# FeatureBaseDB/featurebase

Measured on NVIDIA B200. Metric: set_ops_per_sec, higher is better.
Workload: dtype u64/u16 integer

## Files before the change

### featurebase_b200/csrc/fbgpu.cu

```cuda
#include <cuda_runtime.h>
#include <dlfcn.h>
#include <fcntl.h>
#include <sys/mman.h>
#include <sys/stat.h>
#include <unistd.h>
#include <stdarg.h>
#include <stdio.h>
#include <string.h>

#include <algorithm>
#include <condition_variable>
#include <map>
#include <memory>
#include <mutex>
#include <shared_mutex>
#include <atomic>
#include <deque>
#include <functional>
#include <string>
#include <thread>
#include <unordered_map>
#include <vector>

#include "../../include/fbgpu.h"
// ... 109 lines not shown
    cudaEvent_t ev0 = nullptr, ev1 = nullptr;
    DevBuf d_in, d_counts, d_bitmaps, d_info, d_emit_units, d_emit, d_rows, d_aux;
    PinBuf h_in, h_out;
    bool busy = false;
};

struct fbgpu_ctx {
    int device = 0;
    int sm_count = 148;
    std::shared_mutex store_mu;
    std::map<ViewKey, uint32_t> view_ids;
    std::vector<std::vector<int32_t>> shardmaps;
    std::vector<uint64_t> view_arr, view_other;
    std::vector<uint64_t> view_striped;
    std::vector<HostFrag> frags;
    std::vector<FragHdr> h_frags;
    std::vector<RowEnt> h_rows;
    std::vector<ContDesc> h_descs;
    RawBuf staging;
    uint64_t uploaded = 0;
    uint64_t dead_arena = 0;
    bool meta_dirty = false;
    bool tables_valid = false;
    bool dev_tables_valid = false;
    std::vector<std::pair<uint32_t, uint64_t>> dirty_shards;
    size_t dev_rows = 0, dev_descs = 0, dev_frags = 0;
    bool inspect_only = false;
    std::vector<ViewTab> t_views; std::vector<int32_t> t_flat; std::vector<RowTabEnt> t_rowtab;
    bool stripe_arrays = getenv("FBGPU_ARRAY_SORTED") == nullptr;
    long long unit_batch = [] { const char* e = getenv("FBGPU_UNIT_BATCH"); const long long n = e ? atoll(e) : 0; return n >= 16 ? (n / 16) * 16 : 16384ll; }();
    int gd_ctas_per_sm = 3;
    int pair_ctas_per_sm = 2;
    std::atomic<uint64_t> counters_pair_launches{0};
    DevBuf d_payload, d_views, d_shardmap, d_frags, d_rows, d_descs, d_rowtab;
    PinBuf bounce[2];
    uint32_t n_views_dev = 0;
    fbgpu_stats stats{};
    std::mutex ws_mu; std::condition_variable ws_cv;
    std::vector<std::unique_ptr<Workspace>> wss;
    std::mutex cnt_mu; fbgpu_counters counters{};
    void* comm = nullptr; int n_ranks = 1, rank = 0;
    Mailbox* mbox = nullptr; Mailbox* peers[kMaxRanks] = {}; DevBuf d_peers; bool p2p = false; bool peers_local = false; unsigned long long epoch = 0; std::mutex coll_mu;
    long long p2p_timeout_cycles = [] { const char* e = getenv("FBGPU_P2P_TIMEOUT_MS"); const long long ms = e ? atoll(e) : 2000; return (ms > 0 ? ms : 2000) * 2000000ll; }();
};

static StoreRef store_ref(fbgpu_ctx* c) {
    StoreRef s;
    s.views = (const ViewTab*)c->d_views.p; s.shardmap = (const int32_t*)c->d_shardmap.p; s.frags = (const FragHdr*)c->d_frags.p;
    s.rows = (const RowEnt*)c->d_rows.p; s.descs = (const ContDesc*)c->d_descs.p; s.payload = (const uint8_t*)c->d_payload.p; s.rowtab = (const RowTabEnt*)c->d_rowtab.p; s.n_views = c->n_views_dev;
    return s;
}

extern "C" int fbgpu_init(int32_t device_ordinal, fbgpu_ctx** out) try {
    if (!out) return fail(FBGPU_E_INVALID, "out is null");
    if (device_ordinal == FBGPU_DEVICE_NONE) {
        auto c = new fbgpu_ctx(); c->inspect_only = true; c->device = -1;
        *out = c;
        return FBGPU_OK;
    }
    int n = 0;
    CUDA_TRY(cudaGetDeviceCount(&n));
    if (device_ordinal < 0 || device_ordinal >= n) return fail(FBGPU_E_INVALID, "device ordinal %d out of range (%d devices)", device_ordinal, n);
    CUDA_TRY(cudaSetDevice(device_ordinal));
    auto c = new fbgpu_ctx();
    struct Guard { fbgpu_ctx* c; ~Guard() { if (c) fbgpu_shutdown(c); } } guard{ c };
    c->device = device_ordinal;
// ... 645 lines not shown
    if (!c || !out) return fail(FBGPU_E_INVALID, "null argument");
    std::shared_lock<std::shared_mutex> lk(c->store_mu);
    *out = c->stats;
    return 0;
} FBGPU_CATCH

static int compile_program(fbgpu_ctx* c, uint32_t index, const fbgpu_op* ops, int32_t n_ops, std::vector<DevOp>& out, int& depth) {
    Error err;
    ViewLookup lookup = [c, index](uint32_t field, uint32_t view) { return view_id_locked(c, ViewKey{ index, field, view }, false); };
    int rc = compile(ops, n_ops, lookup, out, depth, err);
    if (rc) return fail(rc, "%s", err.msg);
#ifndef FBGPU_WP_LEGACY_LOOP
    expand_push_row(out);
#endif
    return 0;
}

static void bump(fbgpu_ctx* c, uint64_t launches, float ms) {
    std::lock_guard<std::mutex> lk(c->cnt_mu);
    c->counters.kernel_launches += launches; c->counters.queries++; c->counters.last_query_gpu_ms = ms;
}

static int allreduce_u64(fbgpu_ctx* c, Workspace* w, void* dptr, size_t n) {
    if (!c->comm) return 0;
    std::lock_guard<std::mutex> lk(c->coll_mu);
    int r = g_nccl.AllReduce(dptr, dptr, n, kNcclUint64, kNcclSum, c->comm, w->stream);
    if (r != 0) return fail(FBGPU_E_COMM, "ncclAllReduce failed: %s", g_nccl.GetErrorString ? g_nccl.GetErrorString(r) : "?");
    return 0;
}

static std::vector<int2> find_batches(const std::vector<DevOp>& prog);
static int upload_inputs(Workspace* w, const std::vector<DevOp>& prog, const uint64_t* shards, int64_t n_shards, const DevOp** d_prog, const uint64_t** d_shards) {
    std::vector<int2> batches = find_batches(prog);
    size_t pb = prog.size() * sizeof(DevOp), sb = (size_t)n_shards * 8, bb = batches.size() * sizeof(int2), tot = pb + sb + bb;
    if (w->h_in.ensure(tot + 16)) return FBGPU_E_NOMEM;
    if (w->d_in.ensure(pb + sb + 16)) return FBGPU_E_NOMEM;
    if (w->d_aux.ensure(bb + 16)) return FBGPU_E_NOMEM;
    if (pb) memcpy(w->h_in.p, prog.data(), pb);
    if (sb) memcpy((uint8_t*)w->h_in.p + pb, shards, sb);
    if (bb) memcpy((uint8_t*)w->h_in.p + pb + sb, batches.data(), bb);
    if (pb + sb) CUDA_TRY(cudaMemcpyAsync(w->d_in.p, w->h_in.p, pb + sb, cudaMemcpyHostToDevice, w->stream));
    if (bb) CUDA_TRY(cudaMemcpyAsync(w->d_aux.p, (uint8_t*)w->h_in.p + pb + sb, bb, cudaMemcpyHostToDevice, w->stream));
    *d_prog = (const DevOp*)w->d_in.p; *d_shards = (const uint64_t*)((uint8_t*)w->d_in.p + pb);
    return 0;
}

static std::vector<int2> find_batches(const std::vector<DevOp>& prog) {
    std::vector<int2> b;
    for (size_t k = 0; k < prog.size();) {
        uint8_t o = prog[k].op;
        if (o == D_OR_ROW || o == D_ANDNOT_ROW || o == D_XOR_ROW) { size_t e = k + 1; while (e < prog.size() && prog[e].op == o) e++; b.push_back(make_int2((int)k, (int)e)); k = e; }
        else k++;
    }
    return b;
}

static int launch_eval(fbgpu_ctx* c, Workspace* w, const std::vector<DevOp>& prog, const DevOp* d_prog, int depth, const uint64_t* d_shards, long long n_units, EvalOut out) {
    if (n_units <= 0) return 0;
    const int n_ops = (int)prog.size();
    std::vector<int2> batches = find_batches(prog);
    size_t staged_rows = 0; for (auto& b : batches) staged_rows += (size_t)(b.y - b.x);
    if (!out.info && n_ops <= kWpMaxOps && depth <= kWpMaxDepth && !getenv("FBGPU_NO_WORDPAR")) {
        uint64_t arr = 0, other = 0, striped = 0;
        for (const DevOp& o : prog) if (o.op >= D_PUSH_ROW && o.op <= D_ORANDNOT_ROW && o.op != D_PUSH_EMPTY && o.fv < c->view_arr.size()) { arr += c->view_arr[o.fv]; other += c->view_other[o.fv]; striped += c->view_striped[o.fv]; }
        if (striped == 0 && ((other > 0 && arr * 8 <= other) || getenv("FBGPU_FORCE_WORDPAR") != nullptr)) {
            long long blocks = n_units * kWpBlocksPerUnit;
            long long grid = std::min<long long>(blocks, (long long)c->sm_count * std::max(FBGPU_WP_MIN_BLOCKS, 8) * 2);
            eval_wordpar_kernel<<<(unsigned)grid, kWpThreads, 0, w->stream>>>(store_ref(c), d_prog, n_ops, d_shards, n_units, out);
            CUDA_TRY(cudaGetLastError());
            return 0;
        }
    }
    const bool staged = getenv("FBGPU_STAGED") && n_ops <= kStagedMaxOps && staged_rows >= 4;
    const int2* d_batches = reinterpret_cast<const int2*>(w->d_aux.p);
    if (staged) {
        int ctas = 2;
        if (const char* e = getenv("FBGPU_STAGE_CTAS")) ctas = std::max(1, std::min(4, atoi(e)));
        const size_t per_cta = 233472 / ctas - 1024 - 5888;
        size_t stack = (size_t)(depth + 1) * 8192;
        if (stack + 2 * 8192 <= per_cta) {
            uint32_t stg = (uint32_t)(((per_cta - stack) / 2) & ~size_t(127));
            long long grid = std::min<long long>(n_units, (long long)c->sm_count * ctas);
            size_t smem = stack + 2 * (size_t)stg;
            eval_staged_kernel<<<(unsigned)grid, kEvalThreads, smem, w->stream>>>(store_ref(c), d_prog, n_ops, depth, d_batches, (int)batches.size(), stg, d_shards, n_units, out);
            CUDA_TRY(cudaGetLastError());
            return 0;
        }
    }
    size_t smem = (size_t)(depth + 1) * 8192;
    int per_sm = std::max(1, (int)std::min<size_t>(std::min(FBGPU_EVAL_MIN_BLOCKS, 2048 / kEvalThreads), (227 * 1024) / (smem + 3 * 1024 + 512)));
    long long grid = std::min<long long>(n_units, (long long)c->sm_count * per_sm);
    eval_kernel<<<(unsigned)grid, kEvalThreads, smem, w->stream>>>(store_ref(c), d_prog, n_ops, depth, d_batches, (int)batches.size(), d_shards, n_units, out);
    CUDA_TRY(cudaGetLastError());
    return 0;
}

static bool contiguous_shards(const uint64_t* shards, int64_t n) {
    for (int64_t i = 1; i < n; i++) if (shards[i] != shards[0] + (uint64_t)i) return false;
    return n > 0;
}

static int count_impl(fbgpu_ctx* c, uint32_t index, const fbgpu_op* ops, int32_t n_ops, const uint64_t* shards, int64_t n_shards,
                      uint64_t* out_total, uint64_t* out_per_shard, bool collective) {
    if (!c || !out_total || n_shards < 0 || (n_shards && !shards)) return fail(FBGPU_E_INVALID, "null argument");
    USE_DEVICE(c);
    std::shared_lock<std::shared_mutex> lk;
    int rc = lock_committed(c, lk); if (rc) return rc;
    std::vector<DevOp> prog; int depth = 1;
    rc = compile_program(c, index, ops, n_ops, prog, depth); if (rc) return rc;
    WsLease lease(c); Workspace* w = lease.w;
    const DevOp* d_prog; const uint64_t* d_shards;
    rc = upload_inputs(w, prog, shards, n_shards, &d_prog, &d_shards); if (rc) return rc;
    const size_t nper = out_per_shard ? (size_t)n_shards : 0, nc = 1 + nper + 3;
    if (w->d_counts.ensure(nc * 8)) return FBGPU_E_NOMEM;
    if (w->h_out.ensure(nc * 8)) return FBGPU_E_NOMEM;
    CUDA_TRY(cudaMemsetAsync(w->d_counts.p, 0, nc * 8, w->stream));
    unsigned long long* d_total = (unsigned long long*)w->d_counts.p;
    unsigned long long* d_per = out_per_shard ? d_total + 1 : nullptr;
    long long n_units = (long long)n_shards * kSlotsPerRow;
    std::unique_lock<std::mutex> coll_lk(c->coll_mu, std::defer_lock);
    FuseReduce fr{};
    coll_lk.lock();
    const bool p2p = c->p2p && collective;
    if (!p2p) coll_lk.unlock();
    if (p2p) {
// ... 742 lines not shown
    StoreRef st{};
    st.views = c->t_views.data(); st.shardmap = c->t_flat.data(); st.frags = c->h_frags.data(); st.rows = c->h_rows.data(); st.descs = c->h_descs.data();
    st.payload = c->staging.p; st.rowtab = c->t_rowtab.data(); st.n_views = (uint32_t)c->t_views.size();
    uint32_t fv = index == 0xffffffffu ? field : view_id_locked(c, ViewKey{ index, field, view }, false);
    Resolved r = resolve(st, fv, shard, row, slot);
    *out_type = 0; *out_card = 0; *out_runs = 0; *out_len = 0;
    if (r.ptr == nullptr) return FBGPU_OK;
    *out_type = r.typ; *out_card = r.card; *out_runs = r.cnt;
    const uint64_t bytes = r.typ == kArray ? (((uint64_t)r.card * 2 + 15) & ~15ull) : r.typ == kBitmap ? 8192 : (((uint64_t)r.cnt * 4 + 15) & ~15ull);
    *out_len = bytes;
    if (bytes > cap || !out_payload) return fail(FBGPU_E_NOSPACE, "payload needs %llu bytes", (unsigned long long)bytes);
    if ((const uint8_t*)r.ptr + bytes > c->staging.p + c->staging.len) return fail(FBGPU_E_INVALID, "descriptor points outside the payload arena");
    memcpy(out_payload, r.ptr, bytes);
    return FBGPU_OK;
} FBGPU_CATCH

extern "C" int fbgpu_debug_compile(fbgpu_ctx* c, uint32_t index, const fbgpu_op* ops, int32_t n_ops, uint8_t* out, int32_t cap_ops, int32_t* out_n, int32_t* out_depth) try {
    if (!c || !out_n || !out_depth) return fail(FBGPU_E_INVALID, "null argument");
    std::shared_lock<std::shared_mutex> lk(c->store_mu);
    std::vector<DevOp> prog; int depth = 1;
    int rc = compile_program(c, index, ops, n_ops, prog, depth); if (rc) return rc;
    *out_n = (int32_t)prog.size(); *out_depth = depth;
    if ((int32_t)prog.size() > cap_ops || (!out && !prog.empty())) return fail(FBGPU_E_NOSPACE, "program has %zu ops", prog.size());
    static_assert(sizeof(DevOp) == 16, "DevOp layout");
    if (!prog.empty()) memcpy(out, prog.data(), prog.size() * sizeof(DevOp));
    return FBGPU_OK;
} FBGPU_CATCH

extern "C" int fbgpu_get_counters(fbgpu_ctx* c, fbgpu_counters* out) try {
    if (!c || !out) return fail(FBGPU_E_INVALID, "null argument");
    std::lock_guard<std::mutex> lk(c->cnt_mu);
    *out = c->counters;
    out->pair_kernel_queries = (uint32_t)c->counters_pair_launches.load();
    return 0;
} FBGPU_CATCH
extern "C" void* fbgpu_stream(fbgpu_ctx* c) { return c && !c->wss.empty() ? (void*)c->wss[0]->stream : nullptr; }

extern "C" int fbgpu_rows_payload_bytes(fbgpu_ctx* c, uint32_t index, uint32_t field, uint32_t view, const uint64_t* row_ids, int32_t n_rows,
                                        const uint64_t* shards, int64_t n_shards, uint64_t* out_payload, uint64_t* out_containers) try {
    if (!c || !out_payload || !out_containers) return fail(FBGPU_E_INVALID, "null argument");
    std::shared_lock<std::shared_mutex> lk(c->store_mu);
    uint64_t pay = 0, nc = 0;
    uint32_t fv = view_id_locked(c, ViewKey{ index, field, view }, false);
    if (fv != kNoView) for (int64_t s = 0; s < n_shards; s++) {
        const auto& sm = c->shardmaps[fv];
        if (shards[s] >= sm.size() || sm[shards[s]] < 0) continue;
        const HostFrag& f = c->frags[sm[shards[s]]];
        for (uint32_t k = 0; k < f.n_rows; k++) {
            const RowEnt& e = c->h_rows[f.row_off + k];
            bool want = row_ids == nullptr;
            for (int32_t r = 0; !want && r < n_rows; r++) want = row_ids[r] == e.row;
            if (!want) continue;
            int n = __builtin_popcount(e.mask);
            for (int q = 0; q < n; q++) { const ContDesc& d = c->h_descs[e.first_desc + q]; pay += d.typ == kArray ? 2ull * d.card : d.typ == kBitmap ? 8192 : 4ull * d.cnt; nc++; }
        }
    }
    *out_payload = pay; *out_containers = nc;
    return 0;
} FBGPU_CATCH

#include "node.h"
```

### featurebase_b200/csrc/fbgpu_types.h

```cpp
#pragma once
#include <stdint.h>

namespace fbgpu {

constexpr int kSlotsPerRow = 16;
constexpr int kBitmapWords = 1024;
constexpr uint32_t kFull = 65536;

enum : uint16_t { kArray = 1, kBitmap = 2, kRun = 3 };

struct ContDesc {
    uint32_t off16;
    uint32_t card;
    uint16_t typ;
    uint16_t cnt;
    uint32_t pad;
};

struct RowEnt {
    uint64_t row;
    uint32_t first_desc;
    uint16_t mask;
    uint16_t pad;
};
// ... 19 lines not shown
struct RowTabEnt {
    uint32_t first_desc;
    uint16_t mask;
    uint16_t pad;
};

struct StoreRef {
    const ViewTab* views;
    const int32_t* shardmap;
    const FragHdr* frags;
    const RowEnt* rows;
    const ContDesc* descs;
    const uint8_t* payload;
    const RowTabEnt* rowtab;
    uint32_t n_views;
};

enum : uint8_t {
    D_PUSH_ROW = 1, D_PUSH_EMPTY, D_OR_ROW, D_AND_ROW, D_ANDNOT_ROW, D_XOR_ROW,
    D_ORAND_ROW,
    D_ORANDNOT_ROW,
    D_AND, D_OR, D_ANDNOT, D_XOR,
    D_SWAP, D_POP
};
constexpr uint32_t kNoView = 0xffffffffu;

struct DevOp {
    uint8_t op;
    uint8_t pad[3];
    uint32_t fv;
    uint64_t row;
};

struct Resolved {
    const void* ptr;
    uint32_t card;
    uint16_t typ;
    uint16_t cnt;
};

}
```

### featurebase_b200/csrc/kernels.cuh

```cuda
#pragma once
#include <cuda_runtime.h>
#include <stdint.h>
#include "fbgpu_types.h"
#include "bitaddr.h"
#include "wp_machine.h"
#include "resolve.h"

namespace fbgpu {

#ifndef FBGPU_EVAL_THREADS
#define FBGPU_EVAL_THREADS 256
#endif
#ifndef FBGPU_EVAL_MIN_BLOCKS
#define FBGPU_EVAL_MIN_BLOCKS 6
#endif
constexpr int kEvalThreads = FBGPU_EVAL_THREADS;
constexpr int kEvalU4PerThread = 512 / kEvalThreads;
constexpr int kEvalW64PerThread = 1024 / kEvalThreads;
constexpr int kResolveChunk = 128;

__device__ __forceinline__ uint4 ldg_nc(const uint4* p) {
    uint4 r;
    asm volatile("ld.global.nc.L1::no_allocate.v4.u32 {%0,%1,%2,%3}, [%4];" : "=r"(r.x), "=r"(r.y), "=r"(r.z), "=r"(r.w) : "l"(p));
    return r;
// ... 121 lines not shown
template <int MODE>
__device__ __forceinline__ void smem_bit_op_at(uint32_t addr, uint32_t sh) {
    const uint32_t m = 1u << (sh & 31);
    if (MODE == 0) asm volatile("red.shared.or.b32 [%0], %1;" :: "r"(addr), "r"(m) : "memory");
    else if (MODE == 1) asm volatile("red.shared.and.b32 [%0], %1;" :: "r"(addr), "r"(~m) : "memory");
    else asm volatile("red.shared.xor.b32 [%0], %1;" :: "r"(addr), "r"(m) : "memory");
}
template <int MODE>
__device__ __forceinline__ void scatter_chunk_sb(smem_base_t sb, uint4 v, uint32_t base, uint32_t n) {
    uint32_t w[4] = { v.x, v.y, v.z, v.w };
    if (MODE != 2 || base + 8 <= n) {
#pragma unroll
        for (int q = 0; q < 4; q++) {
            smem_bit_op_at<MODE>(word_addr_lo(sb, w[q]), w[q]);
            smem_bit_op_at<MODE>(word_addr_hi(sb, w[q]), upper16(w[q]));
        }
    } else {
#pragma unroll
        for (int q = 0; q < 4; q++) {
            if (base + 2 * q < n) smem_bit_op_at<MODE>(word_addr_lo(sb, w[q]), w[q]);
            if (base + 2 * q + 1 < n) smem_bit_op_at<MODE>(word_addr_hi(sb, w[q]), w[q] >> 16);
        }
    }
}
template <int MODE>
__device__ __forceinline__ void scatter_chunk_unrolled(uint32_t* bm, uint4 v, uint32_t base, uint32_t n) {
    scatter_chunk_sb<MODE>(smem_base((uint32_t)__cvta_generic_to_shared(bm)), v, base, n);
}
static_assert(sizeof(Resolved) == 16, "batch_rows reads a Resolved with one 16-byte shared load");
#ifndef FBGPU_EVAL_DEEP
#define FBGPU_EVAL_DEEP 3
#endif
template <int MODE>
__device__ __forceinline__ void batch_rows(uint32_t* T32, const Resolved* res, int n) {
    const int lane = threadIdx.x & 31, wid = threadIdx.x >> 5;
    smem_base_t sb = smem_base((uint32_t)__cvta_generic_to_shared(T32));
    pin_base(sb);
    for (int j = wid; j < n; j += kEvalThreads / 32) {
        const uint4 raw = *reinterpret_cast<const uint4*>(res + j);
        const uint4* a4 = reinterpret_cast<const uint4*>(((unsigned long long)raw.y << 32) | raw.x);
        if (a4 == nullptr) continue;
        const uint32_t typ = raw.w & 0xffffu;
        if (typ == kArray) {
            const uint32_t card = raw.z, n8 = (card + 7) >> 3;
            uint4 v[FBGPU_EVAL_DEEP];
#pragma unroll
            for (int q = 0; q < FBGPU_EVAL_DEEP; q++) v[q] = ldg_nc(a4 + min((uint32_t)lane + 32u * q, n8 - 1u));
#pragma unroll
            for (int q = 0; q < FBGPU_EVAL_DEEP; q++) if (lane + 32 * q < n8) scatter_chunk_sb<MODE>(sb, v[q], (lane + 32 * q) * 8, card);
            for (uint32_t i = lane + 32 * FBGPU_EVAL_DEEP; i < n8; i += 32) scatter_chunk_sb<MODE>(sb, ldg_nc(a4 + i), i * 8, card);
        } else if (typ == kBitmap) warp_bitmap_atomic<MODE>(T32, a4, lane);
    }
}
constexpr int kMaxRanks = 16;
struct Mailbox { unsigned long long value[2][kMaxRanks]; unsigned long long flag[2][kMaxRanks]; };
struct FuseReduce {
    Mailbox* const* peers;
    unsigned int* ticket;
    unsigned long long* result;
    unsigned int* error;
    unsigned long long epoch;
    long long timeout_cycles;
    int rank, n_ranks;
};
__device__ __forceinline__ void fused_allreduce_tail(const FuseReduce& fr, unsigned long long* total, unsigned int n_callers) {
    if (fr.peers == nullptr) return;
    __threadfence();
    if (atomicAdd(fr.ticket, 1u) != n_callers - 1) return;
    __threadfence();
    const unsigned long long mine = *reinterpret_cast<volatile unsigned long long*>(total);
    const int par = (int)(fr.epoch & 1ull);
    for (int p = 0; p < fr.n_ranks; p++) *reinterpret_cast<volatile unsigned long long*>(&fr.peers[p]->value[par][fr.rank]) = mine;
    __threadfence_system();
    for (int p = 0; p < fr.n_ranks; p++) *reinterpret_cast<volatile unsigned long long*>(&fr.peers[p]->flag[par][fr.rank]) = fr.epoch;
    __threadfence_system();
    Mailbox* me = fr.peers[fr.rank];
    unsigned long long sum = 0;
    for (int q = 0; q < fr.n_ranks; q++) {
        const long long t0 = clock64();
        while (*reinterpret_cast<volatile unsigned long long*>(&me->flag[par][q]) != fr.epoch) {
            if (clock64() - t0 > fr.timeout_cycles) { *fr.error = 1u + (unsigned int)q; *fr.result = ~0ull; __threadfence_system(); return; }
        }
        __threadfence_system();
        sum += *reinterpret_cast<volatile unsigned long long*>(&me->value[par][q]);
    }
    *fr.result = sum;
}
__global__ void p2p_reduce_only_kernel(FuseReduce fr, unsigned long long* total) { fused_allreduce_tail(fr, total, 1u); }

struct EvalOut {
    unsigned long long* total;
    unsigned long long* per_shard;
    uint4* bitmaps;
    uint2* info;
    FuseReduce fr;
};

__global__ void __launch_bounds__(kEvalThreads, FBGPU_EVAL_MIN_BLOCKS)
eval_kernel(StoreRef st, const DevOp* __restrict__ prog, int n_ops, int depth,
            const int2* __restrict__ batches, int n_batches,
            const uint64_t* __restrict__ shards, long long n_units, EvalOut out) {
    extern __shared__ uint4 smem4[];
    __shared__ __align__(16) Resolved res[kResolveChunk];
    __shared__ uint32_t warp_tmp[kEvalThreads / 32];
    __shared__ uint32_t warp_tmp2[kEvalThreads / 32];
    const int tid = threadIdx.x, lane = tid & 31, wid = tid >> 5;
    unsigned long long cta_total = 0;

    for (long long unit = blockIdx.x; unit < n_units; unit += gridDim.x) {
        const uint64_t shard = shards[unit >> 4];
        const int slot = (int)(unit & 15);
        uint64_t map = 0xFEDCBA9876543210ull;
        int top = -1;
        auto phys = [&](int level) -> uint4* { return smem4 + (size_t)((map >> (4 * level)) & 15u) * 512; };
        auto swap_levels = [&](int a, int b) {
            uint64_t pa = (map >> (4 * a)) & 15u, pb = (map >> (4 * b)) & 15u;
            map &= ~((15ull << (4 * a)) | (15ull << (4 * b)));
            map |= (pb << (4 * a)) | (pa << (4 * b));
        };
        int cur_batch = 0;
        for (int base = 0; base < n_ops; base += kResolveChunk) {
            int chunk = min(kResolveChunk, n_ops - base);
            __syncthreads();
            bool is_run = false;
            if (tid < chunk) {
                DevOp op = prog[base + tid];
                Resolved r; r.ptr = nullptr; r.card = 0; r.typ = 0; r.cnt = 0;
                if (op.op >= D_PUSH_ROW && op.op <= D_ORANDNOT_ROW && op.op != D_PUSH_EMPTY) r = resolve(st, op.fv, shard, op.row, slot);
                res[tid] = r;
                is_run = r.ptr != nullptr && r.typ == kRun;
            }
            const int has_runs = __syncthreads_or(is_run);
            for (int k = 0; k < chunk; k++) {
                const uint8_t opc = prog[base + k].op;
                if (opc == D_PUSH_EMPTY) { top++; bm_zero(phys(top)); __syncthreads(); continue; }
                if (opc == D_SWAP) { swap_levels(top, top - 1); continue; }
                if (opc == D_POP) { top--; continue; }
                if (opc >= D_AND && opc <= D_XOR) {
                    int kind = opc == D_AND ? K_AND : opc == D_OR ? K_OR : opc == D_ANDNOT ? K_ANDNOT : K_XOR;
                    bm_apply_smem(kind, phys(top - 1), nullptr, phys(top));
                    top--; __syncthreads(); continue;
                }
                if (opc == D_OR_ROW || opc == D_ANDNOT_ROW || opc == D_XOR_ROW) {
                    while (cur_batch < n_batches && batches[cur_batch].y <= base + k) cur_batch++;
                    const int e = min(cur_batch < n_batches ? batches[cur_batch].y - base : k + 1, chunk);
                    uint4* T = phys(top);
                    uint32_t* T32 = reinterpret_cast<uint32_t*>(T);
                    if (opc == D_OR_ROW) batch_rows<0>(T32, res + k, e - k);
                    else if (opc == D_ANDNOT_ROW) batch_rows<1>(T32, res + k, e - k);
                    else batch_rows<2>(T32, res + k, e - k);
                    __syncthreads();
                    if (has_runs) for (int j = k; j < e; j++) {
                        const Resolved r = res[j];
                        if (r.ptr == nullptr || r.typ != kRun) continue;
                        uint4* S = phys(depth);
                        bm_expand_runs(S, reinterpret_cast<const uint16_t*>(r.ptr), r.cnt, warp_tmp);
                        bm_apply_smem(opc == D_OR_ROW ? K_OR : opc == D_ANDNOT_ROW ? K_ANDNOT : K_XOR, T, nullptr, S);
                        __syncthreads();
                    }
                    k = e - 1;
                    continue;
                }
                int kind = opc == D_PUSH_ROW ? K_PUSH : opc == D_OR_ROW ? K_OR : opc == D_AND_ROW ? K_AND : opc == D_ANDNOT_ROW ? K_ANDNOT
                         : opc == D_XOR_ROW ? K_XOR : opc == D_ORAND_ROW ? K_ORAND : K_ORANDNOT;
                const Resolved r = res[k];
                if (kind == K_PUSH) top++;
                uint4* T = phys(top);
                uint4* B = (kind == K_ORAND || kind == K_ORANDNOT) ? phys(top - 1) : nullptr;
// ... 1781 lines not shown
```

### featurebase_b200/csrc/program_compiler.h

```cpp
#pragma once
#include <stdarg.h>
#include <stdint.h>
#include <stdio.h>

#include <algorithm>
#include <functional>
#include <vector>

#include "../../include/fbgpu.h"
#include "fbgpu_types.h"
#include "host_error.h"

namespace fbgpu {

using ViewLookup = std::function<uint32_t(uint32_t field, uint32_t view)>;
struct Node { fbgpu_op op; std::vector<int> kids; };

struct Compiler {
    const ViewLookup& lookup; Error& err;
    std::vector<DevOp> out; int depth = 0, max_depth = 0;
    Compiler(const ViewLookup& l, Error& e) : lookup(l), err(e) {}
    uint32_t fv_of(uint32_t field, uint32_t view) { return lookup(field, view); }
    void emit(uint8_t op, uint32_t fv = kNoView, uint64_t row = 0) {
        DevOp d{}; d.op = op; d.fv = fv; d.row = row; out.push_back(d);
// ... 146 lines not shown
    }
};

inline int compile(const fbgpu_op* ops, int32_t n_ops, const ViewLookup& lookup, std::vector<DevOp>& out, int& depth, Error& err) {
    if (n_ops < 0 || (n_ops > 0 && !ops)) return err.set(FBGPU_E_INVALID, "bad program");
    std::vector<Node> nodes; std::vector<int> stack;
    for (int i = 0; i < n_ops; i++) {
        Node n; n.op = ops[i];
        bool nary = n.op.opcode >= FBGPU_OP_INTERSECT && n.op.opcode <= FBGPU_OP_NOT;
        if (nary) {
            uint32_t argc = n.op.argc;
            if (argc > stack.size()) return err.set(FBGPU_E_INVALID, "op %d pops %u operands but only %zu available", i, argc, stack.size());
            n.kids.assign(stack.end() - argc, stack.end()); stack.resize(stack.size() - argc);
        }
        nodes.push_back(std::move(n)); stack.push_back((int)nodes.size() - 1);
    }
    if (stack.size() != 1) return err.set(FBGPU_E_INVALID, "program must leave exactly one result (leaves %zu)", stack.size());
    Compiler cp(lookup, err);
    int rc = cp.gen(nodes, stack[0]); if (rc) return rc;
    if (cp.max_depth > 15) return err.set(FBGPU_E_INVALID, "program needs operand stack depth %d > 15", cp.max_depth);
    out.swap(cp.out); depth = std::max(cp.max_depth, 1);
    return 0;
}

inline void expand_push_row(std::vector<DevOp>& prog) {
    std::vector<DevOp> out; out.reserve(prog.size() + 8);
    for (const DevOp& o : prog) {
        if (o.op == D_PUSH_ROW) { DevOp e{}; e.op = D_PUSH_EMPTY; e.fv = kNoView; out.push_back(e); DevOp r = o; r.op = D_OR_ROW; out.push_back(r); }
        else out.push_back(o);
    }
    prog.swap(out);
}

}
```

### featurebase_b200/lib.py

```python
import ctypes as C
import os
import threading

import numpy as np

_HERE = os.path.dirname(os.path.abspath(__file__))
_LIB = None

OP_ROW, OP_INTERSECT, OP_UNION, OP_DIFFERENCE, OP_XOR, OP_NOT, OP_BSI_RANGE, OP_EMPTY, OP_ALL = range(1, 10)
CMP = {"==": 1, "!=": 2, "<": 3, "<=": 4, ">": 5, ">=": 6, "><": 7}
E_INVALID, E_QUERY, E_FORMAT, E_NOSPACE, E_CUDA, E_NOMEM, E_COMM = -1, -2, -3, -4, -5, -6, -7
DEVICE_NONE = -1


_row_tls = threading.local()


class FbgpuError(RuntimeError):
    def __init__(self, code, msg):
        super().__init__(f"fbgpu error {code}: {msg}")
        self.code = code


class Op(C.Structure):
    _fields_ = [("opcode", C.c_uint32), ("field", C.c_uint32), ("view", C.c_uint32), ("argc", C.c_uint32),
                ("a", C.c_uint64), ("b", C.c_uint64), ("lo", C.c_int64), ("hi", C.c_int64)]


class Stats(C.Structure):
    _fields_ = [(n, C.c_uint64) for n in ("fragments", "containers", "array_containers", "bitmap_containers",
                                           "run_containers", "payload_bytes", "device_bytes", "dead_bytes", "full_commits", "patch_commits")]


class Counters(C.Structure):
    _fields_ = [("kernel_launches", C.c_uint64), ("queries", C.c_uint64), ("last_query_gpu_ms", C.c_float),
                ("pair_kernel_queries", C.c_uint32), ("last_algo_bytes", C.c_uint64),
                ("groupby_units", C.c_uint64), ("groupby_fallback_units", C.c_uint64)]


EXPORTS = ["fbgpu_init", "fbgpu_shutdown", "fbgpu_last_error", "fbgpu_abi_version", "fbgpu_load_fragment",
           "fbgpu_load_fragments", "fbgpu_drop_fragment", "fbgpu_commit", "fbgpu_get_stats", "fbgpu_count", "fbgpu_row",
           "fbgpu_row_counts", "fbgpu_row_counts_per_shard", "fbgpu_groupby", "fbgpu_comm_unique_id", "fbgpu_comm_init", "fbgpu_comm_destroy",
           "fbgpu_get_counters", "fbgpu_stream", "fbgpu_rows_payload_bytes", "fbgpu_count_pairs", "fbgpu_columns", "fbgpu_extract", "fbgpu_load_rbf", "fbgpu_load_rbf_dir", "fbgpu_bsi_minmax", "fbgpu_bsi_sum", "fbgpu_compact", "fbgpu_comm_p2p_handle", "fbgpu_comm_p2p_open", "fbgpu_comm_p2p_disable",
           "fbgpu_any", "fbgpu_pair_types", "fbgpu_node_any", "fbgpu_apply_containers", "fbgpu_node_apply_containers",
           "fbgpu_comm_p2p_open_local", "fbgpu_node_init", "fbgpu_node_shutdown", "fbgpu_node_devices", "fbgpu_node_owner", "fbgpu_node_ctx", "fbgpu_node_load_fragment",
           "fbgpu_node_load_fragments", "fbgpu_node_load_rbf_dir", "fbgpu_node_drop_fragment", "fbgpu_node_commit", "fbgpu_node_get_stats", "fbgpu_node_count", "fbgpu_node_row",
           "fbgpu_node_count_pairs", "fbgpu_node_row_counts", "fbgpu_node_groupby", "fbgpu_node_bsi_sum", "fbgpu_node_bsi_minmax"]


def lib_path():
    return os.environ.get("FBGPU_LIB") or os.path.join(_HERE, "libfbgpu.so")


def load():
    global _LIB
    if _LIB is not None:
        return _LIB
    path = lib_path()
    if not os.path.exists(path):
        raise FileNotFoundError(f"{path} missing: run `python -m featurebase_b200.build` (no CPU fallback exists)")
    L = C.CDLL(path)
    vp, u32, u64, i32, i64 = C.c_void_p, C.c_uint32, C.c_uint64, C.c_int32, C.c_int64
    L.fbgpu_init.argtypes, L.fbgpu_init.restype = [i32, C.POINTER(vp)], C.c_int
    L.fbgpu_shutdown.argtypes, L.fbgpu_shutdown.restype = [vp], None
    L.fbgpu_last_error.argtypes, L.fbgpu_last_error.restype = [], C.c_char_p
    L.fbgpu_abi_version.argtypes, L.fbgpu_abi_version.restype = [], i32
    L.fbgpu_load_fragment.argtypes, L.fbgpu_load_fragment.restype = [vp, u32, u32, u32, u64, vp, u64], C.c_int
    L.fbgpu_load_fragments.argtypes, L.fbgpu_load_fragments.restype = [vp, u32, u32, u32, vp, i64, vp, vp], C.c_int
    L.fbgpu_drop_fragment.argtypes, L.fbgpu_drop_fragment.restype = [vp, u32, u32, u32, u64], C.c_int
    L.fbgpu_apply_containers.argtypes, L.fbgpu_apply_containers.restype = [vp, u32, u32, u32, u64, vp, u64, vp, i64], C.c_int
# ... 121 lines not shown
    def debug_compile(self, index, ops):
        arr = ops_array(ops)
        buf = np.zeros(4096 * 16, dtype=np.uint8)
        n, depth = C.c_int32(0), C.c_int32(0)
        self._check(self.L.fbgpu_debug_compile(self.h, index, arr, len(ops), buf.ctypes.data, 4096, C.byref(n), C.byref(depth)))
        rec = np.frombuffer(buf[: n.value * 16].tobytes(), dtype=np.dtype([("op", "u1"), ("pad", "u1", 3), ("fv", "<u4"), ("row", "<u8")]))
        return [(int(r["op"]), int(r["fv"]), int(r["row"])) for r in rec], depth.value

    def drop_fragment(self, index, field, view, shard):
        self._check(self.L.fbgpu_drop_fragment(self.h, index, field, view, int(shard)))

    def apply_containers(self, index, field, view, shard, data=b"", removed_keys=()):
        data = bytes(data or b"")
        buf = (C.c_uint8 * max(len(data), 1)).from_buffer_copy(data or b"\0")
        rk = _u64arr(list(removed_keys))
        self._check(self.L.fbgpu_apply_containers(self.h, index, field, view, int(shard), buf if data else None, len(data),
                                                  rk.ctypes.data if len(rk) else None, len(rk)))

    def commit(self):
        self._check(self.L.fbgpu_commit(self.h))

    def compact(self):
        self._check(self.L.fbgpu_compact(self.h))

    def stats(self):
        s = Stats()
        self._check(self.L.fbgpu_get_stats(self.h, C.byref(s)))
        return {n: getattr(s, n) for n, _ in Stats._fields_}

    def counters(self):
        s = Counters()
        self._check(self.L.fbgpu_get_counters(self.h, C.byref(s)))
        return {"kernel_launches": s.kernel_launches, "queries": s.queries, "last_query_gpu_ms": s.last_query_gpu_ms, "pair_kernel_queries": s.pair_kernel_queries,
                "groupby_units": s.groupby_units, "groupby_fallback_units": s.groupby_fallback_units}

    def count(self, index, ops, shards, per_shard=False):
        sh = _u64arr(shards)
        arr = ops_array(ops)
        tot = C.c_uint64(0)
        per = np.zeros(len(sh), dtype=np.uint64) if per_shard else None
        self._check(self.L.fbgpu_count(self.h, index, arr, len(ops), sh.ctypes.data, len(sh), C.byref(tot),
                                       per.ctypes.data if per_shard else None))
        return (tot.value, per) if per_shard else tot.value

    def any(self, index, ops, shards):
        sh = _u64arr(shards)
        arr = ops_array(ops)
        out = C.c_int32(0)
        self._check(self.L.fbgpu_any(self.h, index, arr, len(ops), sh.ctypes.data, len(sh), C.byref(out)))
        return bool(out.value)

    def pair_types(self, index, field_a, view_a, row_a, field_b, view_b, row_b, shards):
        sh = _u64arr(shards)
        out = np.zeros(16, dtype=np.uint64)
        self._check(self.L.fbgpu_pair_types(self.h, index, field_a, view_a, int(row_a), field_b, view_b, int(row_b), sh.ctypes.data, len(sh), out.ctypes.data))
        return out.reshape(4, 4)

    def row_into(self, index, ops, shards, buf):
        sh = _u64arr(shards)
        arr = ops_array(ops)
        need, cnt = C.c_uint64(0), C.c_uint64(0)
        rc = self.L.fbgpu_row(self.h, index, arr, len(ops), sh.ctypes.data, len(sh), buf.ctypes.data, len(buf), C.byref(need), C.byref(cnt))
        if rc == E_NOSPACE:
            return need.value, cnt.value, False
        self._check(rc)
        return need.value, cnt.value, True

# ... 202 lines not shown
```

### include/fbgpu.h

```cpp
#ifndef FBGPU_H
#define FBGPU_H
#include <stdint.h>

#ifdef __cplusplus
extern "C" {
#endif

#define FBGPU_ABI_VERSION 2

#define FBGPU_OK 0
#define FBGPU_E_INVALID (-1)
#define FBGPU_E_QUERY (-2)
#define FBGPU_E_FORMAT (-3)
#define FBGPU_E_NOSPACE (-4)
#define FBGPU_E_CUDA (-5)
#define FBGPU_E_NOMEM (-6)
#define FBGPU_E_COMM (-7)

typedef struct fbgpu_ctx fbgpu_ctx;

#define FBGPU_DEVICE_NONE (-1)

int fbgpu_init(int32_t device_ordinal, fbgpu_ctx **out);
void fbgpu_shutdown(fbgpu_ctx *ctx);
// ... 121 lines not shown
                                const uint8_t *roaring, uint64_t nbytes, const uint64_t *removed_keys, int64_t n_removed);
int fbgpu_node_commit(fbgpu_node *node);
int fbgpu_node_get_stats(fbgpu_node *node, fbgpu_stats *out);
int fbgpu_node_count(fbgpu_node *node, uint32_t index, const fbgpu_op *ops, int32_t n_ops,
                     const uint64_t *shards, int64_t n_shards, uint64_t *out_total, uint64_t *out_per_shard);
int fbgpu_node_any(fbgpu_node *node, uint32_t index, const fbgpu_op *ops, int32_t n_ops,
                   const uint64_t *shards, int64_t n_shards, int32_t *out_any);
int fbgpu_node_row(fbgpu_node *node, uint32_t index, const fbgpu_op *ops, int32_t n_ops,
                   const uint64_t *shards, int64_t n_shards, uint8_t *out_buf, uint64_t out_cap, uint64_t *out_len, uint64_t *out_count);
int fbgpu_node_count_pairs(fbgpu_node *node, uint32_t index, uint32_t field_a, uint32_t view_a, const uint64_t *rows_a,
                           uint32_t field_b, uint32_t view_b, const uint64_t *rows_b, int32_t n_pairs,
                           const uint64_t *shards, int64_t n_shards, uint64_t *out_counts);
int fbgpu_node_row_counts(fbgpu_node *node, uint32_t index, uint32_t field, uint32_t view, const uint64_t *row_ids, int32_t n_rows,
                          const fbgpu_op *filter, int32_t n_filter_ops, const uint64_t *shards, int64_t n_shards, uint64_t *out_counts);
int fbgpu_node_groupby(fbgpu_node *node, uint32_t index, const uint32_t *fields, const uint32_t *views, int32_t n_fields,
                       const uint64_t *row_ids_flat, const int32_t *n_rows, const fbgpu_op *filter, int32_t n_filter_ops,
                       const uint64_t *shards, int64_t n_shards, uint64_t *out_counts);
int fbgpu_node_bsi_sum(fbgpu_node *node, uint32_t index, const fbgpu_op *ops, int32_t n_ops, uint32_t field, uint32_t view, int32_t bit_depth,
                       const uint64_t *shards, int64_t n_shards, int64_t *out_sum, uint64_t *out_count);
int fbgpu_node_bsi_minmax(fbgpu_node *node, uint32_t index, const fbgpu_op *ops, int32_t n_ops, uint32_t field, uint32_t view, int32_t bit_depth,
                          const uint64_t *shards, int64_t n_shards, int32_t want_max, int64_t *out_val, uint64_t *out_count);

int fbgpu_debug_compile(fbgpu_ctx *ctx, uint32_t index, const fbgpu_op *ops, int32_t n_ops, uint8_t *out, int32_t cap_ops,
                        int32_t *out_n, int32_t *out_depth);

typedef struct {
    uint64_t kernel_launches;
    uint64_t queries;
    float last_query_gpu_ms;
    uint32_t pair_kernel_queries;
    uint64_t last_algo_bytes;
    uint64_t groupby_units;
    uint64_t groupby_fallback_units;
} fbgpu_counters;
int fbgpu_get_counters(fbgpu_ctx *ctx, fbgpu_counters *out);
int fbgpu_rows_payload_bytes(fbgpu_ctx *ctx, uint32_t index, uint32_t field, uint32_t view, const uint64_t *row_ids, int32_t n_rows,
                             const uint64_t *shards, int64_t n_shards, uint64_t *out_payload, uint64_t *out_containers);
void *fbgpu_stream(fbgpu_ctx *ctx);

#ifdef __cplusplus
}
#endif
#endif
```

Baseline: 183.4 million.

## Fuse consecutive push-empty row batches into one multi-target scatter pass

Adds a host-side planner that finds runs of PUSH_EMPTY followed by same-mode row ops (OR/ANDNOT/XOR) within a resolve chunk. It uploads a per-op target byte so the eval kernel can zero all target stack levels once and let warps scatter every row into its own level in a single pass. This removes the per-group __syncthreads barriers and serial batch processing. It also adds L2 prefetch of upcoming operands. It costs extra smem, extra upload bytes and planner work per query, and it is disabled when runs or 'other' views are present.

```diff
diff --git a/featurebase_b200/csrc/fbgpu.cu b/featurebase_b200/csrc/fbgpu.cu
--- a/featurebase_b200/csrc/fbgpu.cu
+++ b/featurebase_b200/csrc/fbgpu.cu
@@ -165,6 +165,7 @@
     int gd_ctas_per_sm = 3;
     int pair_ctas_per_sm = 2;
     std::atomic<uint64_t> counters_pair_launches{0};
+    std::atomic<uint64_t> counters_multi_batch_launches{0};
     DevBuf d_payload, d_views, d_shardmap, d_frags, d_rows, d_descs, d_rowtab;
     PinBuf bounce[2];
     uint32_t n_views_dev = 0;
@@ -876,13 +877,20 @@
 static std::vector<int2> find_batches(const std::vector<DevOp>& prog);
 static int upload_inputs(Workspace* w, const std::vector<DevOp>& prog, const uint64_t* shards, int64_t n_shards, const DevOp** d_prog, const uint64_t** d_shards) {
     std::vector<int2> batches = find_batches(prog);
-    size_t pb = prog.size() * sizeof(DevOp), sb = (size_t)n_shards * 8, bb = batches.size() * sizeof(int2), tot = pb + sb + bb;
+    std::vector<MultiBatch> multi; std::vector<uint8_t> tgt;
+    plan_multi_batches(prog, kResolveChunk, multi, tgt);
+    const size_t b0 = batches.size() * sizeof(int2), m0 = (b0 + 15) & ~size_t(15), mb = multi.size() * sizeof(MultiBatch);
+    size_t pb = prog.size() * sizeof(DevOp), sb = (size_t)n_shards * 8, bb = multi.empty() ? b0 : m0 + mb + tgt.size(), tot = pb + sb + bb;
     if (w->h_in.ensure(tot + 16)) return FBGPU_E_NOMEM;
     if (w->d_in.ensure(pb + sb + 16)) return FBGPU_E_NOMEM;
     if (w->d_aux.ensure(bb + 16)) return FBGPU_E_NOMEM;
     if (pb) memcpy(w->h_in.p, prog.data(), pb);
     if (sb) memcpy((uint8_t*)w->h_in.p + pb, shards, sb);
-    if (bb) memcpy((uint8_t*)w->h_in.p + pb + sb, batches.data(), bb);
+    if (b0) memcpy((uint8_t*)w->h_in.p + pb + sb, batches.data(), b0);
+    if (!multi.empty()) {
+        memcpy((uint8_t*)w->h_in.p + pb + sb + m0, multi.data(), mb);
+        memcpy((uint8_t*)w->h_in.p + pb + sb + m0 + mb, tgt.data(), tgt.size());
+    }
     if (pb + sb) CUDA_TRY(cudaMemcpyAsync(w->d_in.p, w->h_in.p, pb + sb, cudaMemcpyHostToDevice, w->stream));
     if (bb) CUDA_TRY(cudaMemcpyAsync(w->d_aux.p, (uint8_t*)w->h_in.p + pb + sb, bb, cudaMemcpyHostToDevice, w->stream));
     *d_prog = (const DevOp*)w->d_in.p; *d_shards = (const uint64_t*)((uint8_t*)w->d_in.p + pb);
@@ -931,10 +939,23 @@
             return 0;
         }
     }
+    std::vector<MultiBatch> multi; std::vector<uint8_t> tgt;
+    plan_multi_batches(prog, kResolveChunk, multi, tgt);
+    if (!multi.empty() && getenv("FBGPU_NO_MULTI_BATCH")) multi.clear();
+    for (const MultiBatch& m : multi) {
+        for (int i = m.first; i < m.end; i++)
+            if (prog[i].op != D_PUSH_EMPTY && prog[i].fv < c->view_other.size() && c->view_other[prog[i].fv] != 0) { multi.clear(); break; }
+        if (multi.empty()) break;
+    }
+    const size_t m0 = (batches.size() * sizeof(int2) + 15) & ~size_t(15);
+    const MultiBatch* d_multi = reinterpret_cast<const MultiBatch*>((const uint8_t*)w->d_aux.p + m0);
+    const uint8_t* d_tgt = (const uint8_t*)w->d_aux.p + m0 + multi.size() * sizeof(MultiBatch);
+    if (!multi.empty()) c->counters_multi_batch_launches++;
     size_t smem = (size_t)(depth + 1) * 8192;
     int per_sm = std::max(1, (int)std::min<size_t>(std::min(FBGPU_EVAL_MIN_BLOCKS, 2048 / kEvalThreads), (227 * 1024) / (smem + 3 * 1024 + 512)));
     long long grid = std::min<long long>(n_units, (long long)c->sm_count * per_sm);
-    eval_kernel<<<(unsigned)grid, kEvalThreads, smem, w->stream>>>(store_ref(c), d_prog, n_ops, depth, d_batches, (int)batches.size(), d_shards, n_units, out);
+    eval_kernel<<<(unsigned)grid, kEvalThreads, smem, w->stream>>>(store_ref(c), d_prog, n_ops, depth, d_batches, (int)batches.size(),
+                                                                   d_multi, (int)multi.size(), d_tgt, d_shards, n_units, out);
     CUDA_TRY(cudaGetLastError());
     return 0;
 }
@@ -1743,6 +1764,7 @@
     std::lock_guard<std::mutex> lk(c->cnt_mu);
     *out = c->counters;
     out->pair_kernel_queries = (uint32_t)c->counters_pair_launches.load();
+    out->multi_batch_launches = c->counters_multi_batch_launches.load();
     return 0;
 } FBGPU_CATCH
 extern "C" void* fbgpu_stream(fbgpu_ctx* c) { return c && !c->wss.empty() ? (void*)c->wss[0]->stream : nullptr; }
diff --git a/featurebase_b200/csrc/fbgpu_types.h b/featurebase_b200/csrc/fbgpu_types.h
--- a/featurebase_b200/csrc/fbgpu_types.h
+++ b/featurebase_b200/csrc/fbgpu_types.h
@@ -75,6 +75,10 @@
     uint64_t row;
 };
 
+struct MultiBatch {
+    int32_t first, end, groups, pad;
+};
+
 struct Resolved {
     const void* ptr;
     uint32_t card;
diff --git a/featurebase_b200/csrc/kernels.cuh b/featurebase_b200/csrc/kernels.cuh
--- a/featurebase_b200/csrc/kernels.cuh
+++ b/featurebase_b200/csrc/kernels.cuh
@@ -177,24 +177,56 @@
 #define FBGPU_EVAL_DEEP 3
 #endif
 template <int MODE>
+__device__ __forceinline__ void warp_row_operand(uint32_t* T32, smem_base_t sb, const uint4 raw, int lane) {
+    const uint4* a4 = reinterpret_cast<const uint4*>(((unsigned long long)raw.y << 32) | raw.x);
+    const uint32_t typ = raw.w & 0xffffu;
+    if (typ == kArray) {
+        const uint32_t card = raw.z, n8 = (card + 7) >> 3;
+        uint4 v[FBGPU_EVAL_DEEP];
+#pragma unroll
+        for (int q = 0; q < FBGPU_EVAL_DEEP; q++) v[q] = ldg_nc(a4 + min((uint32_t)lane + 32u * q, n8 - 1u));
+#pragma unroll
+        for (int q = 0; q < FBGPU_EVAL_DEEP; q++) if (lane + 32 * q < n8) scatter_chunk_sb<MODE>(sb, v[q], (lane + 32 * q) * 8, card);
+        for (uint32_t i = lane + 32 * FBGPU_EVAL_DEEP; i < n8; i += 32) scatter_chunk_sb<MODE>(sb, ldg_nc(a4 + i), i * 8, card);
+    } else if (typ == kBitmap) warp_bitmap_atomic<MODE>(T32, a4, lane);
+}
+template <int MODE>
 __device__ __forceinline__ void batch_rows(uint32_t* T32, const Resolved* res, int n) {
     const int lane = threadIdx.x & 31, wid = threadIdx.x >> 5;
     smem_base_t sb = smem_base((uint32_t)__cvta_generic_to_shared(T32));
     pin_base(sb);
     for (int j = wid; j < n; j += kEvalThreads / 32) {
         const uint4 raw = *reinterpret_cast<const uint4*>(res + j);
-        const uint4* a4 = reinterpret_cast<const uint4*>(((unsigned long long)raw.y << 32) | raw.x);
-        if (a4 == nullptr) continue;
-        const uint32_t typ = raw.w & 0xffffu;
-        if (typ == kArray) {
-            const uint32_t card = raw.z, n8 = (card + 7) >> 3;
-            uint4 v[FBGPU_EVAL_DEEP];
-#pragma unroll
-            for (int q = 0; q < FBGPU_EVAL_DEEP; q++) v[q] = ldg_nc(a4 + min((uint32_t)lane + 32u * q, n8 - 1u));
-#pragma unroll
-            for (int q = 0; q < FBGPU_EVAL_DEEP; q++) if (lane + 32 * q < n8) scatter_chunk_sb<MODE>(sb, v[q], (lane + 32 * q) * 8, card);
-            for (uint32_t i = lane + 32 * FBGPU_EVAL_DEEP; i < n8; i += 32) scatter_chunk_sb<MODE>(sb, ldg_nc(a4 + i), i * 8, card);
-        } else if (typ == kBitmap) warp_bitmap_atomic<MODE>(T32, a4, lane);
+        if ((raw.x | raw.y) == 0) continue;
+        warp_row_operand<MODE>(T32, sb, raw, lane);
+    }
+}
+__device__ __forceinline__ void prefetch_l2(const void* p) { asm volatile("prefetch.global.L2 [%0];" :: "l"(p)); }
+__device__ __forceinline__ void warp_prefetch_operand(const uint4 raw, int lane) {
+    const uint8_t* p = reinterpret_cast<const uint8_t*>(((unsigned long long)raw.y << 32) | raw.x);
+    if (p == nullptr) return;
+    const uint32_t typ = raw.w & 0xffffu;
+    const uint32_t bytes = typ == kArray ? ((raw.z + 7) >> 3) * 16u : typ == kBitmap ? 8192u : 0u;
+    for (uint32_t off = (uint32_t)lane * 128u; off < bytes; off += 32u * 128u) prefetch_l2(p + off);
+}
+#ifndef FBGPU_EVAL_MULTI_PF
+#define FBGPU_EVAL_MULTI_PF 1
+#endif
+__device__ __forceinline__ void multi_rows(uint4* smem4, uint64_t map, int top, const Resolved* res, const uint8_t* tgt, int n) {
+    const int lane = threadIdx.x & 31, wid = threadIdx.x >> 5;
+    for (int j = wid; j < n; j += kEvalThreads / 32) {
+        const uint4 raw = *reinterpret_cast<const uint4*>(res + j);
+#if FBGPU_EVAL_MULTI_PF
+        if (j + kEvalThreads / 32 < n) warp_prefetch_operand(*reinterpret_cast<const uint4*>(res + j + kEvalThreads / 32), lane);
+#endif
+        if ((raw.x | raw.y) == 0) continue;
+        const uint32_t t = tgt[j];
+        uint32_t* T32 = reinterpret_cast<uint32_t*>(smem4 + (size_t)((map >> (4 * (top + (int)(t >> 2)))) & 15u) * 512);
+        smem_base_t sb = smem_base((uint32_t)__cvta_generic_to_shared(T32));
+        pin_base(sb);
+        if ((t & 3) == 0) warp_row_operand<0>(T32, sb, raw, lane);
+        else if ((t & 3) == 1) warp_row_operand<1>(T32, sb, raw, lane);
+        else warp_row_operand<2>(T32, sb, raw, lane);
     }
 }
 constexpr int kMaxRanks = 16;
@@ -244,9 +276,11 @@
 __global__ void __launch_bounds__(kEvalThreads, FBGPU_EVAL_MIN_BLOCKS)
 eval_kernel(StoreRef st, const DevOp* __restrict__ prog, int n_ops, int depth,
             const int2* __restrict__ batches, int n_batches,
+            const MultiBatch* __restrict__ multi, int n_multi, const uint8_t* __restrict__ multi_tgt,
             const uint64_t* __restrict__ shards, long long n_units, EvalOut out) {
     extern __shared__ uint4 smem4[];
     __shared__ __align__(16) Resolved res[kResolveChunk];
+    __shared__ uint8_t tgt[kResolveChunk];
     __shared__ uint32_t warp_tmp[kEvalThreads / 32];
     __shared__ uint32_t warp_tmp2[kEvalThreads / 32];
     const int tid = threadIdx.x, lane = tid & 31, wid = tid >> 5;
@@ -263,7 +297,7 @@
             map &= ~((15ull << (4 * a)) | (15ull << (4 * b)));
             map |= (pb << (4 * a)) | (pa << (4 * b));
         };
-        int cur_batch = 0;
+        int cur_batch = 0, cur_multi = 0;
         for (int base = 0; base < n_ops; base += kResolveChunk) {
             int chunk = min(kResolveChunk, n_ops - base);
             __syncthreads();
@@ -273,12 +307,29 @@
                 Resolved r; r.ptr = nullptr; r.card = 0; r.typ = 0; r.cnt = 0;
                 if (op.op >= D_PUSH_ROW && op.op <= D_ORANDNOT_ROW && op.op != D_PUSH_EMPTY) r = resolve(st, op.fv, shard, op.row, slot);
                 res[tid] = r;
+                if (n_multi) tgt[tid] = multi_tgt[base + tid];
                 is_run = r.ptr != nullptr && r.typ == kRun;
             }
             const int has_runs = __syncthreads_or(is_run);
             for (int k = 0; k < chunk; k++) {
                 const uint8_t opc = prog[base + k].op;
-                if (opc == D_PUSH_EMPTY) { top++; bm_zero(phys(top)); __syncthreads(); continue; }
+                if (opc == D_PUSH_EMPTY) {
+                    while (cur_multi < n_multi && multi[cur_multi].first < base + k) cur_multi++;
+                    if (cur_multi < n_multi && multi[cur_multi].first == base + k && !has_runs) {
+                        const MultiBatch mb = multi[cur_multi];
+#if FBGPU_EVAL_MULTI_PF
+                        if (wid < mb.end - mb.first) warp_prefetch_operand(*reinterpret_cast<const uint4*>(res + k + wid), lane);
+#endif
+                        for (int l = 1; l <= mb.groups; l++) bm_zero(phys(top + l));
+                        __syncthreads();
+                        multi_rows(smem4, map, top, res + k, tgt + k, mb.end - mb.first);
+                        __syncthreads();
+                        top += mb.groups;
+                        k = mb.end - base - 1;
+                        continue;
+                    }
+                    top++; bm_zero(phys(top)); __syncthreads(); continue;
+                }
                 if (opc == D_SWAP) { swap_levels(top, top - 1); continue; }
                 if (opc == D_POP) { top--; continue; }
                 if (opc >= D_AND && opc <= D_XOR) {
diff --git a/featurebase_b200/csrc/program_compiler.h b/featurebase_b200/csrc/program_compiler.h
--- a/featurebase_b200/csrc/program_compiler.h
+++ b/featurebase_b200/csrc/program_compiler.h
@@ -202,4 +202,27 @@
     prog.swap(out);
 }
 
-}
+inline void plan_multi_batches(const std::vector<DevOp>& prog, int chunk, std::vector<MultiBatch>& out, std::vector<uint8_t>& tgt) {
+    out.clear(); tgt.assign(prog.size(), 0);
+    const int n = (int)prog.size();
+    auto row_mode = [](uint8_t o) { return o == D_OR_ROW ? 0 : o == D_ANDNOT_ROW ? 1 : o == D_XOR_ROW ? 2 : -1; };
+    for (int k = 0; k < n;) {
+        int e = k, groups = 0;
+        while (e + 1 < n && prog[e].op == D_PUSH_EMPTY && row_mode(prog[e + 1].op) >= 0) {
+            int f = e + 1;
+            while (f < n && prog[f].op == prog[e + 1].op) f++;
+            if ((f - 1) / chunk != k / chunk) break;
+            groups++; e = f;
+        }
+        if (groups < 2) { k++; continue; }
+        int g = 0;
+        for (int i = k; i < e; i++) {
+            if (prog[i].op == D_PUSH_EMPTY) g++;
+            else tgt[i] = (uint8_t)(g << 2 | row_mode(prog[i].op));
+        }
+        out.push_back(MultiBatch{ k, e, groups, 0 });
+        k = e;
+    }
+}
+
+}
diff --git a/featurebase_b200/lib.py b/featurebase_b200/lib.py
--- a/featurebase_b200/lib.py
+++ b/featurebase_b200/lib.py
@@ -35,7 +35,8 @@
 class Counters(C.Structure):
     _fields_ = [("kernel_launches", C.c_uint64), ("queries", C.c_uint64), ("last_query_gpu_ms", C.c_float),
                 ("pair_kernel_queries", C.c_uint32), ("last_algo_bytes", C.c_uint64),
-                ("groupby_units", C.c_uint64), ("groupby_fallback_units", C.c_uint64)]
+                ("groupby_units", C.c_uint64), ("groupby_fallback_units", C.c_uint64),
+                ("multi_batch_launches", C.c_uint64)]
 
 
 EXPORTS = ["fbgpu_init", "fbgpu_shutdown", "fbgpu_last_error", "fbgpu_abi_version", "fbgpu_load_fragment",
@@ -223,7 +224,8 @@
         s = Counters()
         self._check(self.L.fbgpu_get_counters(self.h, C.byref(s)))
         return {"kernel_launches": s.kernel_launches, "queries": s.queries, "last_query_gpu_ms": s.last_query_gpu_ms, "pair_kernel_queries": s.pair_kernel_queries,
-                "groupby_units": s.groupby_units, "groupby_fallback_units": s.groupby_fallback_units}
+                "groupby_units": s.groupby_units, "groupby_fallback_units": s.groupby_fallback_units,
+                "multi_batch_launches": s.multi_batch_launches}
 
     def count(self, index, ops, shards, per_shard=False):
         sh = _u64arr(shards)
diff --git a/include/fbgpu.h b/include/fbgpu.h
--- a/include/fbgpu.h
+++ b/include/fbgpu.h
@@ -177,6 +177,7 @@
     uint64_t last_algo_bytes;
     uint64_t groupby_units;
     uint64_t groupby_fallback_units;
+    uint64_t multi_batch_launches;
 } fbgpu_counters;
 int fbgpu_get_counters(fbgpu_ctx *ctx, fbgpu_counters *out);
 int fbgpu_rows_payload_bytes(fbgpu_ctx *ctx, uint32_t index, uint32_t field, uint32_t view, const uint64_t *row_ids, int32_t n_rows,
```

Result: slower. 165.1 million (median of 6 runs) (-10.0%).
